# rgiordan/LinearResponseVariationalBayes.py

Hardware: AMD Instinct MI355X
Metric: ELBO-Hessian builds/sec, N=1e+06 obs x D=1024 free params (higher is better)
Workload: dtype f64

## Files before the change

### linearresponsevariationalbayes.py_amd/csrc/k_wsyrk.hip

```cpp
#include "lrvb_internal.h"
#include <type_traits>
#include <math.h>

typedef double d4 __attribute__((ext_vector_type(4)));
typedef double d2 __attribute__((ext_vector_type(2)));

constexpr int WS_LDS_STRIDE = WS_TILE + 16;

int wsyrk_num_tiles(i64 P) {
    i64 nb = (P + WS_TILE - 1) / WS_TILE;
    return (int)(nb * (nb + 1) / 2);
}

int wsyrk_auto_splits(const lrvb_ctx* c) {
    if (c->n_splits_user > 0) return ((c->n_splits_user + 7) / 8) * 8;
    int T = wsyrk_num_tiles(c->P);
    i64 s = (4608 + T / 2) / T;
    s = ((s + 7) / 8) * 8;
    i64 max_by_rows = c->N / 1900;
    max_by_rows = (max_by_rows / 8) * 8;
    if (s > max_by_rows) s = max_by_rows;
    if (s > 128) s = 128;
    if (s < 8) s = 8;
    return (int)s;
// ... 593 lines not shown

    d4 acc[16];
#pragma unroll
    for (int i = 0; i < 16; ++i) acc[i] = (d4){0.0, 0.0, 0.0, 0.0};
    int ca = bi * WS_TILE + 2 * lane; if (ca > PA - 2) ca = PA - 2;
    int cb = bj * WS_TILE + 2 * lane; if (cb > PB - 2) cb = PB - 2;

    const unsigned lds0 = (unsigned)(uintptr_t)(__attribute__((address_space(3))) double*)lds;
    const unsigned voffA = (unsigned)ca * 8u, voffB = (unsigned)cb * 8u, voffC = (unsigned)lane * 4u;
    const unsigned voffX = (unsigned)(lane < 62 ? lane : 61) * 4u;
    auto issue_stage = [&](int ch, int buf) {
        const unsigned base = lds0 + (unsigned)(buf * WS_BUF) * 8u;
        const i64 n0 = r0 + (i64)ch * WS_KC;
#pragma unroll
        for (int i = 0; i < 4; ++i) {
            const int row = wave + 4 * i;
            i64 n = n0 + row; if (n > N - 1) n = N - 1;
            const unsigned la = base + (unsigned)(row * WS_LDS_STRIDE) * 8u;
            if (SLIVER == 2)
                WS_GLDS4_S(reinterpret_cast<const char*>(A + n * lda), voffX, la + 8u);
            else
                WS_GLDS16_S(reinterpret_cast<const char*>(A + n * lda), voffA, la);
            WS_GLDS16_S(reinterpret_cast<const char*>(B + n * ldb), voffB, la + (unsigned)WS_PANEL * 8u);
        }
        if (wave == 0)
            WS_GLDS4_S(reinterpret_cast<const char*>(cpad + n0), voffC, base + (unsigned)(2 * WS_PANEL) * 8u);
    };
    if (SLIVER == 2) {
        if (tid < 32) lds[(tid >> 4) * WS_BUF + (tid & 15) * WS_LDS_STRIDE] = 1.0;
        __syncthreads();
    }
    if (nch > 0) issue_stage(0, 0);
    __builtin_amdgcn_s_waitcnt(0x0F70);
    __syncthreads();

    const int l15 = lane & 15, l4 = lane >> 4;
    const int wr = wave >> 1, wc = wave & 1;
    int mt_a = (PA - bi * WS_TILE - wr * 64 + 15) / 16; mt_a = mt_a < 0 ? 0 : (mt_a > 4 ? 4 : mt_a);
    int mt_b = (PB - bj * WS_TILE - wc * 64 + 15) / 16; mt_b = mt_b < 0 ? 0 : (mt_b > 4 ? 4 : mt_b);
    mt_a = __builtin_amdgcn_readfirstlane(mt_a); mt_b = __builtin_amdgcn_readfirstlane(mt_b);
    const bool full = (PA - bi * WS_TILE >= WS_TILE) && (PB - bj * WS_TILE >= WS_TILE);
    double* out = partial + ((i64)split * T + t) * (i64)(WS_TILE * WS_TILE);
    if (full) {
        const double* a_base = lds + l4 * WS_LDS_STRIDE + 32 * wave + 2 * l15;
        const double* b_base = lds + WS_PANEL + l4 * WS_LDS_STRIDE + 2 * l15;
        const double* c_base = lds + 2 * WS_PANEL + l4;
        const double* a_base_s = a_base + bj * 4 * WS_LDS_STRIDE;
        const double* b_base_s = b_base + bi * 4 * WS_LDS_STRIDE + 32 * wave;
        const double* c_base_i = c_base + bj * 4;
        const double* c_base_ii = c_base + bi * 4;
        const unsigned voffSA = (unsigned)(((i64)(4 * bi + l4) * lda + 4 * WS_TILE + l15) * 8);
        const unsigned voffSB = (unsigned)(((i64)(4 * bj + l4) * ldb + 4 * WS_TILE + l15) * 8);
        double asl[2] = {0.0, 0.0}, bsl[2] = {0.0, 0.0};
        d4 acc_i0 = (d4){0.0, 0.0, 0.0, 0.0}, acc_i1 = acc_i0, acc_ii0 = acc_i0, acc_ii1 = acc_i0, acc_c = acc_i0;
        auto pair_of = [](int v, int& a, int& b) {
            a = (int)((sqrtf(8.f * (float)v + 1.f) - 1.f) * 0.5f);
            while (a * (a + 1) / 2 > v) --a;
            while ((a + 1) * (a + 2) / 2 <= v) ++a;
            b = v - a * (a + 1) / 2;
        };
        const double *ga0 = lds, *gb0 = lds, *ga1 = lds, *gb1 = lds, *gas = lds, *gbs = lds;
        if (SLIVER == 2) {
            int a, b;
            pair_of(bi * WS_TILE + 32 * wave + 2 * l15, a, b);     ga0 = lds + l4 * WS_LDS_STRIDE + a; gb0 = lds + l4 * WS_LDS_STRIDE + b;
            pair_of(bi * WS_TILE + 32 * wave + 2 * l15 + 1, a, b); ga1 = lds + l4 * WS_LDS_STRIDE + a; gb1 = lds + l4 * WS_LDS_STRIDE + b;
            pair_of(4 * WS_TILE + l15, a, b);
            gas = lds + (4 * bi + l4) * WS_LDS_STRIDE + a; gbs = lds + (4 * bi + l4) * WS_LDS_STRIDE + b;
        }
        const bool corner = SLIVER && (bi == bj) && (wave == 0);
        auto load_sliver = [&](int ch, double& a, double& b) {
            const i64 n0 = r0 + (i64)ch * WS_KC;
            if (SLIVER == 1) asm volatile("global_load_dwordx2 %0, %1, %2" : "+v"(a) : "v"(voffSA), "s"(A + n0 * lda) : "memory");
            asm volatile("global_load_dwordx2 %0, %1, %2" : "+v"(b) : "v"(voffSB), "s"(B + n0 * ldb) : "memory");
        };
        if (SLIVER) {
            load_sliver(0, asl[0], bsl[0]);
            __builtin_amdgcn_s_waitcnt(0x0F70);
            asm volatile("" : "+v"(asl[0]), "+v"(bsl[0]));
        }
        auto stage = [&](auto buf_tag, int ch) {
            constexpr int BUF = decltype(buf_tag)::value;
            double af[2][2], gf[2][2], bf[2][8], cv[2];
            if (SLIVER) load_sliver(ch + 1 < nch ? ch + 1 : ch, asl[BUF ^ 1], bsl[BUF ^ 1]);
            d2 ax = (d2){0.0, 0.0}, bx = (d2){0.0, 0.0};
            double cxi = 0.0, cxii = 0.0;
            double asg = 0.0;
            if (SLIVER) {
                if (SLIVER == 2) {
                    const int os = BUF * WS_BUF + bj * 4 * WS_LDS_STRIDE;
                    ax = (d2){ga0[os] * gb0[os], ga1[os] * gb1[os]};
                    asg = gas[BUF * WS_BUF] * gbs[BUF * WS_BUF];
                } else {
                    ax = *reinterpret_cast<const d2*>(a_base_s + BUF * WS_BUF);
                }
                bx = *reinterpret_cast<const d2*>(b_base_s + BUF * WS_BUF);
                cxi = c_base_i[BUF * WS_BUF]; cxii = c_base_ii[BUF * WS_BUF];
            }
            auto read_frags = [&](int kk, int set) {
                const int o = BUF * WS_BUF + kk * 4 * WS_LDS_STRIDE;
                cv[set] = c_base[BUF * WS_BUF + kk * 4];
                if (SLIVER == 2) {
                    af[set][0] = ga0[o]; af[set][1] = ga1[o]; gf[set][0] = gb0[o]; gf[set][1] = gb1[o];
                } else {
                    const d2 va = *reinterpret_cast<const d2*>(a_base + o);
                    af[set][0] = va[0]; af[set][1] = va[1];
                }
#pragma unroll
                for (int h = 0; h < 4; ++h) {
                    const d2 vb = *reinterpret_cast<const d2*>(b_base + o + 32 * h);
                    bf[set][2 * h] = vb[0]; bf[set][2 * h + 1] = vb[1];
                }
            };
            read_frags(0, 0);
#pragma unroll
            for (int kk = 0; kk < WS_KC / 4; ++kk) {
                const int set = kk & 1;
                const double as0 = (SLIVER == 2 ? af[set][0] * gf[set][0] : af[set][0]) * cv[set];
                const double as1 = (SLIVER == 2 ? af[set][1] * gf[set][1] : af[set][1]) * cv[set];
                __builtin_amdgcn_sched_barrier(0);
                if (kk + 1 < WS_KC / 4) read_frags(kk + 1, set ^ 1);
                __builtin_amdgcn_sched_barrier(0);
#pragma unroll
                for (int n = 0; n < 8; ++n) {
                    acc[n] = __builtin_amdgcn_mfma_f64_16x16x4f64(as0, bf[set][n], acc[n], 0, 0, 0);
                    acc[8 + n] = __builtin_amdgcn_mfma_f64_16x16x4f64(as1, bf[set][n], acc[8 + n], 0, 0, 0);
                }
                if (SLIVER && kk == 1) {
                    const double sa = (SLIVER == 2 ? asg : asl[BUF]) * cxii;
                    acc_i0 = __builtin_amdgcn_mfma_f64_16x16x4f64(ax[0] * cxi, bsl[BUF], acc_i0, 0, 0, 0);
                    acc_i1 = __builtin_amdgcn_mfma_f64_16x16x4f64(ax[1] * cxi, bsl[BUF], acc_i1, 0, 0, 0);
                    acc_ii0 = __builtin_amdgcn_mfma_f64_16x16x4f64(sa, bx[0], acc_ii0, 0, 0, 0);
                    acc_ii1 = __builtin_amdgcn_mfma_f64_16x16x4f64(sa, bx[1], acc_ii1, 0, 0, 0);
                    if (corner) acc_c = __builtin_amdgcn_mfma_f64_16x16x4f64(sa, bsl[BUF], acc_c, 0, 0, 0);
                }
                __builtin_amdgcn_sched_barrier(0);
            }
            __builtin_amdgcn_s_waitcnt(0x0F70);
            if (SLIVER) asm volatile("" : "+v"(asl[BUF ^ 1]), "+v"(bsl[BUF ^ 1]));
            __syncthreads();
        };
        for (int ch = 0; ch < nch; ch += 2) {
            if (ch + 1 < nch) issue_stage(ch + 1, 1);
            stage(std::integral_constant<int, 0>{}, ch);
            if (ch + 1 < nch) {
                if (ch + 2 < nch) issue_stage(ch + 2, 0);
                stage(std::integral_constant<int, 1>{}, ch + 1);
            }
        }
#pragma unroll
        for (int m = 0; m < 2; ++m)
#pragma unroll
            for (int n = 0; n < 8; ++n)
#pragma unroll
                for (int r = 0; r < 4; ++r)
                    out[(32 * wave + 2 * (l4 + 4 * r) + m) * WS_TILE + 32 * (n >> 1) + 2 * l15 + (n & 1)] = acc[m * 8 + n][r];
        if (SLIVER) {
            double* oe = partial + ((i64)split * T + (bi * nbb + 4)) * (i64)(WS_TILE * WS_TILE);
            double* of = partial + ((i64)split * T + (4 * nbb + bj)) * (i64)(WS_TILE * WS_TILE);
#pragma unroll
            for (int r = 0; r < 4; ++r) {
                oe[(32 * wave + 2 * (l4 + 4 * r)) * WS_TILE + 16 * bj + l15] = acc_i0[r];
                oe[(32 * wave + 2 * (l4 + 4 * r) + 1) * WS_TILE + 16 * bj + l15] = acc_i1[r];
                of[(16 * bi + l4 + 4 * r) * WS_TILE + 32 * wave + 2 * l15] = acc_ii0[r];
                of[(16 * bi + l4 + 4 * r) * WS_TILE + 32 * wave + 2 * l15 + 1] = acc_ii1[r];
            }
            if (corner) {
                double* oc = partial + ((i64)split * T + (4 * nbb + 4)) * (i64)(WS_TILE * WS_TILE);
#pragma unroll
                for (int r = 0; r < 4; ++r) oc[(16 * bi + l4 + 4 * r) * WS_TILE + l15] = acc_c[r];
            }
        }
        return;
    }
    int buf = 0;
    for (int ch = 0; ch < nch; ++ch) {
        if (ch + 1 < nch) issue_stage(ch + 1, buf ^ 1);
        const double* As = lds + buf * WS_BUF;
        const double* Bs = As + WS_PANEL;
        const double* Cs = As + 2 * WS_PANEL;
        double af[2][4], bf[2][4], cv[2];
        auto read_frags = [&](int kk, int set) {
            const int krow = kk * 4 + l4;
            cv[set] = Cs[krow];
#pragma unroll
            for (int m = 0; m < 4; ++m) af[set][m] = As[krow * WS_LDS_STRIDE + wr * 64 + m * 16 + l15];
#pragma unroll
            for (int n = 0; n < 4; ++n) bf[set][n] = Bs[krow * WS_LDS_STRIDE + wc * 64 + n * 16 + l15];
        };
        read_frags(0, 0);
#pragma unroll
        for (int kk = 0; kk < WS_KC / 4; ++kk) {
            const int set = kk & 1;
            double as[4];
#pragma unroll
            for (int m = 0; m < 4; ++m) as[m] = af[set][m] * cv[set];
            __builtin_amdgcn_sched_barrier(0);
            if (kk + 1 < WS_KC / 4) read_frags(kk + 1, set ^ 1);
            __builtin_amdgcn_sched_barrier(0);
#pragma unroll
            for (int m = 0; m < 4; ++m)
#pragma unroll
                for (int n = 0; n < 4; ++n)
                    if (m < mt_a && n < mt_b)
                        acc[m * 4 + n] = __builtin_amdgcn_mfma_f64_16x16x4f64(as[m], bf[set][n], acc[m * 4 + n], 0, 0, 0);
            __builtin_amdgcn_sched_barrier(0);
        }
        __builtin_amdgcn_s_waitcnt(0x0F70);
        __syncthreads();
        buf ^= 1;
    }
#pragma unroll
    for (int m = 0; m < 4; ++m)
#pragma unroll
        for (int n = 0; n < 4; ++n)
#pragma unroll
            for (int r = 0; r < 4; ++r)
                out[(wr * 64 + m * 16 + l4 + 4 * r) * WS_TILE + wc * 64 + n * 16 + l15] = acc[m * 4 + n][r];
}

int launch_atb_kron32(lrvb_ctx* c, const double* X31, const double* B, i64 N, const double* cvec_dev, double* C_dev);

__global__ __launch_bounds__(256)
void atb_tiles_to_dense_kernel(const double* __restrict__ tiles, int nbb, i64 PA, i64 PB, double* __restrict__ C, i64 ldc, int sliver)
{
    const i64 j = (i64)blockIdx.x * blockDim.x + threadIdx.x;
    const i64 i = blockIdx.y;
    if (j >= PB || i >= PA) return;
    const i64 ti = i / WS_TILE, tj = j / WS_TILE, li = i % WS_TILE, lj = j % WS_TILE;
    const double* tile = tiles + (ti * nbb + tj) * (WS_TILE * WS_TILE);
    if (!sliver || (ti < 4 && tj < 4)) { C[i * ldc + j] = tile[li * WS_TILE + lj]; return; }
    double s = 0.0;
    if (ti < 4)      for (int g = 0; g < 4; ++g) s += tile[li * WS_TILE + 16 * g + lj];
    else             for (int g = 0; g < 4; ++g) s += tile[(16 * g + li) * WS_TILE + lj];
    C[i * ldc + j] = s;
}

int launch_atb(lrvb_ctx* c, const double* A, i64 PA, const double* B, i64 PB, i64 N,
               const double* cvec_dev, double* C_dev, bool rows_padded) {
    if ((PA % 2) || (PB % 2) || (((uintptr_t)A) & 15) || (((uintptr_t)B) & 15))
        LRVB_FAIL(LRVB_ERR_UNSUPPORTED, "atb: operands must have even widths and 16-byte aligned rows");
    const int nba = (int)((PA + WS_TILE - 1) / WS_TILE), nbb = (int)((PB + WS_TILE - 1) / WS_TILE);
    const int T = nba * nbb;
    const bool sliver = rows_padded && PA == 4 * WS_TILE + 16 && PB == 4 * WS_TILE + 16;
    const int TW = sliver ? 16 : T;
    i64 S = (4608 + TW / 2) / TW;
    S = ((S + 7) / 8) * 8;
    i64 max_by_rows = (N / 256 / 8) * 8;
    if (S > max_by_rows) S = max_by_rows;
    if (S > 128) S = 128;
    if (S < 8) S = 8;
    i64 rps = (N + S - 1) / S;
    rps = ((rps + WS_KC - 1) / WS_KC) * WS_KC;
    const i64 tile_elems = (i64)T * WS_TILE * WS_TILE;
    LRVB_TRY(buf_reserve(c, c->tile_part, (size_t)(tile_elems * (S + 1))));
    double* part = c->tile_part.p;
    double* tiles = c->tile_part.p + tile_elems * S;
    if (c->prof_on) LRVB_TRY(prof_mark(c, PROF_WSYRK));
    if (sliver)
        hipLaunchKernelGGL(atb_glds_kernel<1>, dim3((unsigned)(S * 16)), dim3(WS_THREADS), 0, c->stream,
                           A, PA, (int)PA, B, PB, (int)PB, N, cvec_dev, (int)S, nba, nbb, rps, part);
    else
        hipLaunchKernelGGL(atb_glds_kernel<0>, dim3((unsigned)(S * T)), dim3(WS_THREADS), 0, c->stream,
                           A, PA, (int)PA, B, PB, (int)PB, N, cvec_dev, (int)S, nba, nbb, rps, part);
    HIP_TRY(hipGetLastError());
    if (c->prof_on) LRVB_TRY(prof_mark(c, PROF_WSYRK));
    hipLaunchKernelGGL(wsyrk_reduce_kernel, dim3((unsigned)((tile_elems / 2 + 255) / 256)), dim3(256), 0, c->stream,
                       part, (int)S, tile_elems, tiles);
    HIP_TRY(hipGetLastError());
    dim3 grid((unsigned)((PB + 255) / 256), (unsigned)PA);
    hipLaunchKernelGGL(atb_tiles_to_dense_kernel, grid, dim3(256), 0, c->stream, tiles, nbb, PA, PB, C_dev, PB, sliver ? 1 : 0);
    HIP_TRY(hipGetLastError());
    return LRVB_OK;
}


int launch_atb_kron32(lrvb_ctx* c, const double* X31, const double* B, i64 N, const double* cvec_dev, double* C_dev) {
    const i64 PA = 4 * WS_TILE + 16, PB = PA;
    if ((((uintptr_t)B) & 15) || (((uintptr_t)X31) & 7)) LRVB_FAIL(LRVB_ERR_UNSUPPORTED, "atb: operand alignment");
    const int nba = 5, nbb = 5, T = 25;
    i64 S = 128;
    i64 max_by_rows = (N / 256 / 8) * 8;
    if (S > max_by_rows) S = max_by_rows;
    if (S < 8) S = 8;
    i64 rps = (N + S - 1) / S;
    rps = ((rps + WS_KC - 1) / WS_KC) * WS_KC;
    const i64 tile_elems = (i64)T * WS_TILE * WS_TILE;
    LRVB_TRY(buf_reserve(c, c->tile_part, (size_t)(tile_elems * (S + 1))));
    double* part = c->tile_part.p;
    double* tiles = c->tile_part.p + tile_elems * S;
    if (c->prof_on) LRVB_TRY(prof_mark(c, PROF_WSYRK));
    hipLaunchKernelGGL(atb_glds_kernel<2>, dim3((unsigned)(S * 16)), dim3(WS_THREADS), 0, c->stream,
                       X31, (i64)31, (int)PA, B, PB, (int)PB, N, cvec_dev, (int)S, nba, nbb, rps, part);
    HIP_TRY(hipGetLastError());
    if (c->prof_on) LRVB_TRY(prof_mark(c, PROF_WSYRK));
    hipLaunchKernelGGL(wsyrk_reduce_kernel, dim3((unsigned)((tile_elems / 2 + 255) / 256)), dim3(256), 0, c->stream,
                       part, (int)S, tile_elems, tiles);
    HIP_TRY(hipGetLastError());
    dim3 grid((unsigned)((PB + 255) / 256), (unsigned)PA);
    hipLaunchKernelGGL(atb_tiles_to_dense_kernel, grid, dim3(256), 0, c->stream, tiles, nbb, PA, PB, C_dev, PB, 1);
    HIP_TRY(hipGetLastError());
    return LRVB_OK;
}

constexpr int KR_STRIDE = 176;
constexpr int KR_ZERO = 65;
constexpr int KR_CZ = 80;

__device__ __forceinline__ void kr_pair(int v, int pv, int& a, int& b) {
    if (v >= pv) { a = KR_ZERO; b = KR_ZERO; return; }
    a = (int)((sqrtf(8.f * (float)v + 1.f) - 1.f) * 0.5f);
    while (a * (a + 1) / 2 > v) --a;
    while ((a + 1) * (a + 2) / 2 <= v) ++a;
    b = v - a * (a + 1) / 2;
}

__global__ __launch_bounds__(WS_THREADS, 2)
void wsyrk_kron_kernel(const double* __restrict__ Z, i64 ldz, i64 N, int q, int pv,
                       const double* __restrict__ cpad, int n_splits, int nb, i64 rows_per_split,
                       double* __restrict__ partial)
{
    __shared__ double lds[2 * WS_KC * KR_STRIDE];
    const int tid = threadIdx.x;
    const int lane = tid & 63;
    const int wave = __builtin_amdgcn_readfirstlane(tid >> 6);
    const int xcd = blockIdx.x & 7;
    const int qpos = blockIdx.x >> 3;
    const int S8 = n_splits >> 3;
    const int n_off = nb * (nb - 1) / 2;
    int bi, bj, split_local;
    if (qpos < n_off * S8) {
        split_local = qpos / n_off;
        const int u = qpos - split_local * n_off;
        bi = (int)((1.f + sqrtf(1.f + 8.f * (float)u)) * 0.5f);
        while (bi * (bi - 1) / 2 > u) --bi;
        while ((bi + 1) * bi / 2 <= u) ++bi;
        bj = u - bi * (bi - 1) / 2;
    } else {
        const int qd = qpos - n_off * S8;
        split_local = qd / nb;
        bi = bj = qd - split_local * nb;
    }
    const bool diag = (bi == bj);
    const int t = bi * (bi + 1) / 2 + bj;
    const int T = nb * (nb + 1) / 2;
    const int split = split_local * 8 + xcd;
    i64 r0 = (i64)split * rows_per_split;
    i64 r1 = r0 + rows_per_split;
    if (r1 > N) r1 = N;
    if (r0 > N) r0 = N;
    const int nch = (int)((r1 - r0 + WS_KC - 1) / WS_KC);

    d4 acc[16];
#pragma unroll
    for (int i = 0; i < 16; ++i) acc[i] = (d4){0.0, 0.0, 0.0, 0.0};

    const int srow = tid >> 4, seg = tid & 15;
    double sv[4], sc;
    auto load_stage = [&](int ch) {
        i64 n = r0 + (i64)ch * WS_KC + srow;
        sc = cpad[n];
        if (n > N - 1) n = N - 1;
        const double* rowp = Z + n * ldz;
#pragma unroll
        for (int j = 0; j < 4; ++j) { const int col = 4 * seg + j; sv[j] = rowp[col < q ? col : 0]; }
    };
    auto store_stage = [&](int buf) {
        asm volatile("" : "+v"(sv[0]), "+v"(sv[1]), "+v"(sv[2]), "+v"(sv[3]), "+v"(sc));
        double* dst = lds + buf * (WS_KC * KR_STRIDE) + srow * KR_STRIDE;
#pragma unroll
        for (int j = 0; j < 4; ++j) { const int col = 4 * seg + j; const double zv = col < q ? sv[j] : 0.0; dst[col] = zv; dst[KR_CZ + col] = zv * sc; }
    };
    if (tid < 2 * WS_KC) { lds[tid * KR_STRIDE + KR_ZERO] = 0.0; lds[tid * KR_STRIDE + KR_CZ + KR_ZERO] = 0.0; }

    if (nch > 0) { load_stage(0); store_stage(0); }
    __syncthreads();

    const int l15 = lane & 15, l4 = lane >> 4;
    int buf = 0;
    if (!diag) {
        const int wr = wave >> 1, wc = wave & 1;
        int ia[4], ib[4], ja[4], jb[4];
#pragma unroll
        for (int m = 0; m < 4; ++m) {
            kr_pair(bi * WS_TILE + wr * 64 + 16 * m + l15, pv, ia[m], ib[m]);
            kr_pair(bj * WS_TILE + wc * 64 + 16 * m + l15, pv, ja[m], jb[m]);
        }
        int mt_a = (pv - (bi * WS_TILE + wr * 64) + 15) / 16;
        mt_a = __builtin_amdgcn_readfirstlane(mt_a < 0 ? 0 : (mt_a > 4 ? 4 : mt_a));
        for (int ch = 0; ch < nch; ++ch) {
            const bool more = ch + 1 < nch;
            if (more) load_stage(ch + 1);
            const double* zs = lds + buf * (WS_KC * KR_STRIDE);
            double xa[2][4], xb[2][4], ya[2][4], yb[2][4];
            auto read_frags = [&](int kk, int set) {
                const double* rowp = zs + (kk * 4 + l4) * KR_STRIDE;
#pragma unroll
                for (int m = 0; m < 4; ++m) { xa[set][m] = rowp[KR_CZ + ia[m]]; xb[set][m] = rowp[ib[m]]; ya[set][m] = rowp[ja[m]]; yb[set][m] = rowp[jb[m]]; }
            };
            read_frags(0, 0);
#pragma unroll
            for (int kk = 0; kk < WS_KC / 4; ++kk) {
                const int set = kk & 1;
                double af[4], bf[4];
#pragma unroll
                for (int m = 0; m < 4; ++m) { af[m] = xa[set][m] * xb[set][m]; bf[m] = ya[set][m] * yb[set][m]; }
                __builtin_amdgcn_sched_barrier(0);
                if (kk + 1 < WS_KC / 4) read_frags(kk + 1, set ^ 1);
                __builtin_amdgcn_sched_barrier(0);
                __builtin_amdgcn_s_setprio(1);
#pragma unroll
                for (int m = 0; m < 4; ++m)
#pragma unroll
                    for (int n = 0; n < 4; ++n)
                        if (m < mt_a)
                            acc[m * 4 + n] = __builtin_amdgcn_mfma_f64_16x16x4f64(af[m], bf[n], acc[m * 4 + n], 0, 0, 0);
                __builtin_amdgcn_s_setprio(0);
                __builtin_amdgcn_sched_barrier(0);
            }
            if (more) store_stage(buf ^ 1);
            __syncthreads();
            buf ^= 1;
        }
        double* out = partial + ((i64)split * T + t) * (i64)(WS_TILE * WS_TILE);
#pragma unroll
        for (int m = 0; m < 4; ++m)
#pragma unroll
            for (int n = 0; n < 4; ++n)
#pragma unroll
                for (int r = 0; r < 4; ++r)
                    out[(wr * 64 + m * 16 + l4 + 4 * r) * WS_TILE + wc * 64 + n * 16 + l15] = acc[m * 4 + n][r];
    } else {
        const int rb0 = wave, rb1 = 7 - wave;
        const int nreal = (pv - bi * WS_TILE + 15) / 16;
        int i0a, i0b, i1a, i1b, ja[8], jb[8];
        kr_pair(bi * WS_TILE + 16 * rb0 + l15, pv, i0a, i0b);
        kr_pair(bi * WS_TILE + 16 * rb1 + l15, pv, i1a, i1b);
#pragma unroll
        for (int n = 0; n < 8; ++n) kr_pair(bi * WS_TILE + 16 * n + l15, pv, ja[n], jb[n]);
        for (int ch = 0; ch < nch; ++ch) {
            const bool more = ch + 1 < nch;
            if (more) load_stage(ch + 1);
            const double* zs = lds + buf * (WS_KC * KR_STRIDE);
            double ya[2][8], yb[2][8], a0[2], a1[2];
            auto read_frags = [&](int kk, int set) {
                const double* rowp = zs + (kk * 4 + l4) * KR_STRIDE;
#pragma unroll
                for (int n = 0; n < 8; ++n) { ya[set][n] = rowp[ja[n]]; yb[set][n] = rowp[jb[n]]; }
                a0[set] = rowp[KR_CZ + i0a] * rowp[i0b];
                a1[set] = rowp[KR_CZ + i1a] * rowp[i1b];
            };
            read_frags(0, 0);
#pragma unroll
            for (int kk = 0; kk < WS_KC / 4; ++kk) {
                const int set = kk & 1;
                double bf[8];
#pragma unroll
                for (int n = 0; n < 8; ++n) bf[n] = ya[set][n] * yb[set][n];
                const double af0 = a0[set], af1 = a1[set];
                __builtin_amdgcn_sched_barrier(0);
                if (kk + 1 < WS_KC / 4) read_frags(kk + 1, set ^ 1);
                __builtin_amdgcn_sched_barrier(0);
#pragma unroll
                for (int n = 0; n < 4; ++n)
                    if (n <= rb0 && rb0 < nreal) acc[n] = __builtin_amdgcn_mfma_f64_16x16x4f64(af0, bf[n], acc[n], 0, 0, 0);
#pragma unroll
                for (int n = 0; n < 8; ++n)
                    if (n <= rb1 && rb1 < nreal) acc[4 + n] = __builtin_amdgcn_mfma_f64_16x16x4f64(af1, bf[n], acc[4 + n], 0, 0, 0);
                __builtin_amdgcn_sched_barrier(0);
            }
            if (more) store_stage(buf ^ 1);
            __syncthreads();
            buf ^= 1;
        }
        double* out = partial + ((i64)split * T + t) * (i64)(WS_TILE * WS_TILE);
#pragma unroll
        for (int n = 0; n < 8; ++n)
#pragma unroll
            for (int r = 0; r < 4; ++r) {
                const double v0 = (n < 4 && n <= rb0) ? acc[n < 4 ? n : 0][r] : 0.0;
                const double v1 = (n <= rb1) ? acc[4 + n][r] : 0.0;
                out[(rb0 * 16 + l4 + 4 * r) * WS_TILE + n * 16 + l15] = v0;
                out[(rb1 * 16 + l4 + 4 * r) * WS_TILE + n * 16 + l15] = v1;
            }
    }
}

int launch_wsyrk_kron(lrvb_ctx* c, const double* cvec_dev, double* tiles_out_dev) {
    const int q = (int)c->P;
    if (q > 64) LRVB_FAIL(LRVB_ERR_UNSUPPORTED, "Kronecker Gram kernel supports n_cols <= 64 (got %d)", q);
    const int pv = q * (q + 1) / 2;
    const int nb = (pv + WS_TILE - 1) / WS_TILE;
    const int T = nb * (nb + 1) / 2;
    i64 S = (9216 + T / 2) / T;
    S = ((S + 7) / 8) * 8;
    i64 max_by_rows = (c->N / 256 / 8) * 8;
    if (S > max_by_rows) S = max_by_rows;
    if (S > 128) S = 128;
    if (S < 8) S = 8;
    i64 rps = (c->N + S - 1) / S;
    rps = ((rps + WS_KC - 1) / WS_KC) * WS_KC;
    const i64 tile_elems = (i64)T * WS_TILE * WS_TILE;
    LRVB_TRY(buf_reserve(c, c->tile_part, (size_t)(tile_elems * S)));
    if (c->prof_on) LRVB_TRY(prof_mark(c, PROF_WSYRK));
    hipLaunchKernelGGL(wsyrk_kron_kernel, dim3((unsigned)(S * T)), dim3(WS_THREADS), 0, c->stream,
                       c->X.p, c->P, c->N, q, pv, cvec_dev, (int)S, nb, rps, c->tile_part.p);
    HIP_TRY(hipGetLastError());
    if (c->prof_on) LRVB_TRY(prof_mark(c, PROF_WSYRK));
    const i64 nthreads = tile_elems / 2;
    hipLaunchKernelGGL(wsyrk_reduce_kernel, dim3((unsigned)((nthreads + 255) / 256)), dim3(256), 0, c->stream,
                       c->tile_part.p, (int)S, tile_elems, tiles_out_dev);
    HIP_TRY(hipGetLastError());
    if (c->prof_on) {
        const double pvd = (double)pv;
        c->prof.wsyrk_flops = (double)c->N * pvd * (pvd + 1.0);
        c->prof.wsyrk_bytes = 8.0 * (double)c->N * (q + 1.0) + 8.0 * 0.5 * pvd * (pvd + 1.0);
    }
    return LRVB_OK;
}

__global__ __launch_bounds__(256)
void wsyrk_reduce_kernel(const double* __restrict__ partial, int n_splits, i64 tile_elems_total,
                         double* __restrict__ tiles)
{
    const i64 e2 = ((i64)blockIdx.x * blockDim.x + threadIdx.x) * 2;
    if (e2 >= tile_elems_total) return;
    double s0 = 0.0, s1 = 0.0;
    typedef double v2d __attribute__((ext_vector_type(2)));
    for (int s = 0; s < n_splits; ++s) {
        const v2d v = __builtin_nontemporal_load(reinterpret_cast<const v2d*>(partial + (i64)s * tile_elems_total + e2));
        s0 += v[0]; s1 += v[1];
    }
    *reinterpret_cast<double2*>(tiles + e2) = make_double2(s0, s1);
}

__global__ __launch_bounds__(512)
void rpart_reduce_kernel(const double* __restrict__ rpart, int n_splits, i64 width, i64 P, double* __restrict__ r)
{
    __shared__ double sh[8][64];
    const int cx = threadIdx.x & 63, ry = threadIdx.x >> 6;
    const i64 p = (i64)blockIdx.x * 64 + cx;
    double s0 = 0.0, s1 = 0.0;
    if (p < P) {
        int k = ry;
        for (; k + 8 < n_splits; k += 16) { s0 += rpart[(i64)k * width + p]; s1 += rpart[(i64)(k + 8) * width + p]; }
        for (; k < n_splits; k += 8) s0 += rpart[(i64)k * width + p];
    }
    sh[ry][cx] = s0 + s1;
    __syncthreads();
    if (ry == 0 && p < P) {
        double t = sh[0][cx];
#pragma unroll
        for (int g = 1; g < 8; ++g) t += sh[g][cx];
        r[p] = t;
    }
}

bool wsyrk_fast_path(const lrvb_ctx* c) {
    return c->P > 64 && (c->P % 2) == 0 && ((((uintptr_t)c->X.p) & 15) == 0) && !c->force_generic_wsyrk;
}

int launch_wsyrk(lrvb_ctx* c, const double* cvec_dev, double* tiles_out_dev) {
    return launch_wsyrk_r(c, cvec_dev, tiles_out_dev, nullptr, nullptr);
}

int launch_wsyrk_r(lrvb_ctx* c, const double* cvec_dev, double* tiles_out_dev, const double* cy_dev, double* r_out_dev) {
    if (cy_dev && !wsyrk_fast_path(c)) LRVB_FAIL(LRVB_ERR_UNSUPPORTED, "the column sums ride on the LDS-DMA SYRK kernel only");
    if (c->P <= 64 && !c->force_generic_wsyrk)
        return launch_gram_small(c, cvec_dev, tiles_out_dev);
    const int T = wsyrk_num_tiles(c->P);
    const int S = wsyrk_auto_splits(c);
    i64 rps = (c->N + S - 1) / S;
    rps = ((rps + WS_KC - 1) / WS_KC) * WS_KC;
    if (rps < WS_KC) rps = WS_KC;
    const i64 tile_elems = (i64)T * WS_TILE * WS_TILE;
    const int nbt = (int)((c->P + WS_TILE - 1) / WS_TILE);
    const i64 rwidth = (i64)nbt * WS_TILE;
    LRVB_TRY(buf_reserve(c, c->tile_part, (size_t)(tile_elems * S) + (size_t)(rwidth * S)));
    double* rpart = c->tile_part.p + tile_elems * S;
    const i64 ldx = c->P;
    const int vec_ok = ((ldx % 2) == 0) && ((((uintptr_t)c->X.p) & 15) == 0);
    const int grid = S * T;
    if (c->prof_on) LRVB_TRY(prof_mark(c, PROF_WSYRK));
    if (vec_ok && c->P >= 2 && !c->force_generic_wsyrk)
        hipLaunchKernelGGL(wsyrk_glds_kernel, dim3(grid), dim3(WS_THREADS), 0, c->stream,
                           c->X.p, ldx, c->N, (int)c->P, cvec_dev, S, nbt, rps, c->tile_part.p, cy_dev, rpart);
    else if (vec_ok)
        hipLaunchKernelGGL(wsyrk_kernel<true>, dim3(grid), dim3(WS_THREADS), 0, c->stream,
                           c->X.p, ldx, c->N, (int)c->P, cvec_dev, S, T, rps, c->tile_part.p);
    else
        hipLaunchKernelGGL(wsyrk_kernel<false>, dim3(grid), dim3(WS_THREADS), 0, c->stream,
                           c->X.p, ldx, c->N, (int)c->P, cvec_dev, S, T, rps, c->tile_part.p);
    HIP_TRY(hipGetLastError());
    if (c->prof_on) LRVB_TRY(prof_mark(c, PROF_WSYRK));
    const i64 nthreads = tile_elems / 2;
    hipLaunchKernelGGL(wsyrk_reduce_kernel, dim3((unsigned)((nthreads + 255) / 256)), dim3(256), 0, c->stream,
                       c->tile_part.p, S, tile_elems, tiles_out_dev);
    HIP_TRY(hipGetLastError());
    if (cy_dev && r_out_dev) {
        hipLaunchKernelGGL(rpart_reduce_kernel, dim3((unsigned)((c->P + 63) / 64)), dim3(512), 0, c->stream,
                           rpart, S, rwidth, c->P, r_out_dev);
        HIP_TRY(hipGetLastError());
    }
    if (c->prof_on) {
        c->prof.wsyrk_flops = (double)c->N * (double)c->P * (double)(c->P + 1);
        c->prof.wsyrk_bytes = 8.0 * ((double)c->N * (double)(c->P + 1)) + 8.0 * 0.5 * (double)c->P * (double)(c->P + 1);
    }
    return LRVB_OK;
}

__global__ __launch_bounds__(256)
void tiles_to_dense_kernel(const double* __restrict__ tiles, i64 P, double* __restrict__ dense,
                           i64 ld, i64 row_off, i64 col_off, int accumulate)
{
    const i64 j = (i64)blockIdx.x * blockDim.x + threadIdx.x;
    const i64 i = blockIdx.y;
    if (j >= P || i >= P) return;
    const i64 a = i > j ? i : j, b = i > j ? j : i;
    const i64 ba = a / WS_TILE, bb = b / WS_TILE;
    const i64 t = ba * (ba + 1) / 2 + bb;
    const double v = tiles[t * (WS_TILE * WS_TILE) + (a % WS_TILE) * WS_TILE + (b % WS_TILE)];
    double* dst = dense + (row_off + i) * ld + col_off + j;
    if (accumulate) *dst += v; else *dst = v;
}

int launch_tiles_to_dense(lrvb_ctx* c, const double* tiles_dev, i64 P, double* dense_dev, i64 ld,
                          i64 row_off, i64 col_off, bool accumulate) {
    if (P <= 0) return LRVB_OK;
    dim3 grid((unsigned)((P + 255) / 256), (unsigned)P);
    hipLaunchKernelGGL(tiles_to_dense_kernel, grid, dim3(256), 0, c->stream,
                       tiles_dev, P, dense_dev, ld, row_off, col_off, accumulate ? 1 : 0);
    HIP_TRY(hipGetLastError());
    return LRVB_OK;
}

__global__ __launch_bounds__(256)
void wsyrk_batched_reduce_kernel(const double* __restrict__ partial, int n_splits, i64 tile_elems, double* __restrict__ tiles)
{
    const i64 e = (i64)blockIdx.x * blockDim.x + threadIdx.x;
    if (e >= tile_elems) return;
    const i64 g = blockIdx.y;
    const double* src = partial + g * (i64)n_splits * tile_elems + e;
    double s = 0.0;
    for (int k = 0; k < n_splits; ++k) s += __builtin_nontemporal_load(src + (i64)k * tile_elems);
    tiles[g * tile_elems + e] = s;
}

bool wsyrk_batched_supported(const lrvb_ctx* c) { return wsyrk_fast_path(c); }

int launch_wsyrk_batched(lrvb_ctx* c, const double* cols, i64 cstride, int G, double* tiles_out) {
    if (!wsyrk_batched_supported(c)) LRVB_FAIL(LRVB_ERR_UNSUPPORTED, "batched SYRK: even P > 64, 16-byte aligned X");
    if (G <= 0) return LRVB_OK;
    const int T = wsyrk_num_tiles(c->P);
    const i64 Teff = (i64)T * G;
    i64 S = (4608 + Teff / 2) / Teff;
    S = ((S + 7) / 8) * 8;
    i64 max_by_rows = (c->N / 1900 / 8) * 8;
    if (S > max_by_rows) S = max_by_rows;
    if (S > 128) S = 128;
    if (S < 8) S = 8;
    i64 rps = (c->N + S - 1) / S;
    rps = ((rps + WS_KC - 1) / WS_KC) * WS_KC;
    if (rps < WS_KC) rps = WS_KC;
    const i64 tile_elems = (i64)T * WS_TILE * WS_TILE;
    LRVB_TRY(buf_reserve(c, c->tile_part, (size_t)(tile_elems * S * G)));
    const int nbt = (int)((c->P + WS_TILE - 1) / WS_TILE);
    if (c->prof_on) LRVB_TRY(prof_mark(c, PROF_WSYRK));
    hipLaunchKernelGGL(wsyrk_glds_batched_kernel, dim3((unsigned)(S * T), (unsigned)G), dim3(WS_THREADS), 0, c->stream,
                       c->X.p, c->P, c->N, (int)c->P, cols, cstride, (int)S, nbt, rps, c->tile_part.p, tile_elems * S);
    HIP_TRY(hipGetLastError());
    if (c->prof_on) LRVB_TRY(prof_mark(c, PROF_WSYRK));
    hipLaunchKernelGGL(wsyrk_batched_reduce_kernel, dim3((unsigned)((tile_elems + 255) / 256), (unsigned)G), dim3(256), 0, c->stream,
                       (const double*)c->tile_part.p, (int)S, tile_elems, tiles_out);
    HIP_TRY(hipGetLastError());
    return LRVB_OK;
}
```

Baseline: 65.11.

## Pre-form Kronecker product panels in LDS with a three-stage pipeline

The Kronecker Gram kernel now has each wave gather raw Z row entries and compute the pairwise products once per row into packed LDS panels, rather than every MFMA lane recomputing products from scattered LDS reads. A pipeline runs global load, raw-row staging, and panel formation for the next chunk while MFMAs consume the current panel. Fragment reads become vectorised d2 loads, and full chunks use precomputed byte offsets instead of per-row clamping. The cost is more LDS, more pipeline bookkeeping, and a reworked wave-to-output mapping that must remain correct for partial tiles.

```diff
diff --git a/linearresponsevariationalbayes.py_amd/csrc/k_wsyrk.hip b/linearresponsevariationalbayes.py_amd/csrc/k_wsyrk.hip
--- a/linearresponsevariationalbayes.py_amd/csrc/k_wsyrk.hip
+++ b/linearresponsevariationalbayes.py_amd/csrc/k_wsyrk.hip
@@ -919,12 +919,16 @@
     return LRVB_OK;
 }
 
-constexpr int KR_STRIDE = 176;
-constexpr int KR_ZERO = 65;
-constexpr int KR_CZ = 80;
+constexpr int KP_PANEL = WS_KC * WS_TILE;
+constexpr int KP_BUF = 2 * KP_PANEL;
+constexpr int KZ_STRIDE = 82;
+constexpr int KZ_ZERO = 64;
+constexpr int KZ_C = 66;
+constexpr int KZ_BASE = 2 * KP_BUF;
+constexpr int KR_LDS = KZ_BASE + WS_KC * KZ_STRIDE;
 
 __device__ __forceinline__ void kr_pair(int v, int pv, int& a, int& b) {
-    if (v >= pv) { a = KR_ZERO; b = KR_ZERO; return; }
+    if (v >= pv) { a = KZ_ZERO; b = KZ_ZERO; return; }
     a = (int)((sqrtf(8.f * (float)v + 1.f) - 1.f) * 0.5f);
     while (a * (a + 1) / 2 > v) --a;
     while ((a + 1) * (a + 2) / 2 <= v) ++a;
@@ -936,7 +940,7 @@
                        const double* __restrict__ cpad, int n_splits, int nb, i64 rows_per_split,
                        double* __restrict__ partial)
 {
-    __shared__ double lds[2 * WS_KC * KR_STRIDE];
+    __shared__ __attribute__((aligned(16))) double lds[KR_LDS];
     const int tid = threadIdx.x;
     const int lane = tid & 63;
     const int wave = __builtin_amdgcn_readfirstlane(tid >> 6);
@@ -971,125 +975,186 @@
 #pragma unroll
     for (int i = 0; i < 16; ++i) acc[i] = (d4){0.0, 0.0, 0.0, 0.0};
 
-    const int srow = tid >> 4, seg = tid & 15;
+    const int srow = 4 * wave + (lane >> 4), seg = lane & 15;
+    unsigned zoff[4];
+#pragma unroll
+    for (int j = 0; j < 4; ++j) { const int col = 4 * seg + j; zoff[j] = (unsigned)(((i64)srow * ldz + (col < q ? col : 0)) * 8); }
+    const unsigned coff = (unsigned)srow * 8u;
+    i64 full = (N - r0) / WS_KC;
+    const int nch_full = (int)(full < nch ? full : nch);
     double sv[4], sc;
     auto load_stage = [&](int ch) {
-        i64 n = r0 + (i64)ch * WS_KC + srow;
-        sc = cpad[n];
-        if (n > N - 1) n = N - 1;
-        const double* rowp = Z + n * ldz;
-#pragma unroll
-        for (int j = 0; j < 4; ++j) { const int col = 4 * seg + j; sv[j] = rowp[col < q ? col : 0]; }
+        const i64 n0 = r0 + (i64)ch * WS_KC;
+        if (ch < nch_full) {
+            const char* zb = reinterpret_cast<const char*>(Z) + n0 * ldz * 8;
+            const char* cb = reinterpret_cast<const char*>(cpad + n0);
+#pragma unroll
+            for (int j = 0; j < 4; ++j) sv[j] = *reinterpret_cast<const double*>(zb + zoff[j]);
+            sc = *reinterpret_cast<const double*>(cb + coff);
+        } else {
+            i64 n = n0 + srow;
+            sc = cpad[n < N ? n : N];
+            if (n > N - 1) n = N - 1;
+            const char* zb = reinterpret_cast<const char*>(Z) + (n - srow) * ldz * 8;
+#pragma unroll
+            for (int j = 0; j < 4; ++j) sv[j] = *reinterpret_cast<const double*>(zb + zoff[j]);
+        }
     };
-    auto store_stage = [&](int buf) {
+    double* zrow_w = lds + KZ_BASE + srow * KZ_STRIDE;
+    auto store_stage = [&]() {
         asm volatile("" : "+v"(sv[0]), "+v"(sv[1]), "+v"(sv[2]), "+v"(sv[3]), "+v"(sc));
-        double* dst = lds + buf * (WS_KC * KR_STRIDE) + srow * KR_STRIDE;
-#pragma unroll
-        for (int j = 0; j < 4; ++j) { const int col = 4 * seg + j; const double zv = col < q ? sv[j] : 0.0; dst[col] = zv; dst[KR_CZ + col] = zv * sc; }
+        *reinterpret_cast<d2*>(zrow_w + 4 * seg) = (d2){sv[0], sv[1]};
+        *reinterpret_cast<d2*>(zrow_w + 4 * seg + 2) = (d2){sv[2], sv[3]};
+        zrow_w[KZ_C + seg] = sc;
     };
-    if (tid < 2 * WS_KC) { lds[tid * KR_STRIDE + KR_ZERO] = 0.0; lds[tid * KR_STRIDE + KR_CZ + KR_ZERO] = 0.0; }
-
-    if (nch > 0) { load_stage(0); store_stage(0); }
+    if (lane < 4) lds[KZ_BASE + (4 * wave + lane) * KZ_STRIDE + KZ_ZERO] = 0.0;
+
+    const double* zw = lds + KZ_BASE + 4 * wave * KZ_STRIDE;
+    const double *ga[4], *gb[4];
+    {
+        int a, b;
+#pragma unroll
+        for (int e = 0; e < 4; ++e) {
+            kr_pair((e < 2 ? bi : bj) * WS_TILE + 64 * (e & 1) + lane, pv, a, b);
+            ga[e] = zw + a; gb[e] = zw + b;
+        }
+    }
+    const double* gc = zw + KZ_C;
+    double* pw = lds + 4 * wave * WS_TILE + 2 * lane;
+    double g[8], gck;
+    auto gather = [&](int row) {
+        if (!diag) {
+#pragma unroll
+            for (int e = 0; e < 4; ++e) { g[2 * e] = ga[e][row * KZ_STRIDE]; g[2 * e + 1] = gb[e][row * KZ_STRIDE]; }
+        } else {
+#pragma unroll
+            for (int e = 0; e < 2; ++e) { g[2 * e] = ga[e][row * KZ_STRIDE]; g[2 * e + 1] = gb[e][row * KZ_STRIDE]; }
+        }
+        gck = gc[row * KZ_STRIDE];
+    };
+    auto form = [&](int row, int nbuf) {
+        double* dst = pw + nbuf * KP_BUF + row * WS_TILE;
+        if (!diag) {
+            *reinterpret_cast<d2*>(dst) = (d2){(g[0] * g[1]) * gck, (g[2] * g[3]) * gck};
+            *reinterpret_cast<d2*>(dst + KP_PANEL) = (d2){g[4] * g[5], g[6] * g[7]};
+        } else {
+            *reinterpret_cast<d2*>(dst) = (d2){g[0] * g[1], g[2] * g[3]};
+            dst[KP_PANEL - lane] = gck;
+        }
+    };
+
+    load_stage(0); store_stage();
     __syncthreads();
+#pragma unroll
+    for (int row = 0; row < 4; ++row) { gather(row); form(row, 0); }
+    load_stage(1); store_stage();
+    __syncthreads();
 
     const int l15 = lane & 15, l4 = lane >> 4;
-    int buf = 0;
+    double* out = partial + ((i64)split * T + t) * (i64)(WS_TILE * WS_TILE);
     if (!diag) {
-        const int wr = wave >> 1, wc = wave & 1;
-        int ia[4], ib[4], ja[4], jb[4];
-#pragma unroll
-        for (int m = 0; m < 4; ++m) {
-            kr_pair(bi * WS_TILE + wr * 64 + 16 * m + l15, pv, ia[m], ib[m]);
-            kr_pair(bj * WS_TILE + wc * 64 + 16 * m + l15, pv, ja[m], jb[m]);
-        }
-        int mt_a = (pv - (bi * WS_TILE + wr * 64) + 15) / 16;
-        mt_a = __builtin_amdgcn_readfirstlane(mt_a < 0 ? 0 : (mt_a > 4 ? 4 : mt_a));
-        for (int ch = 0; ch < nch; ++ch) {
-            const bool more = ch + 1 < nch;
-            if (more) load_stage(ch + 1);
-            const double* zs = lds + buf * (WS_KC * KR_STRIDE);
-            double xa[2][4], xb[2][4], ya[2][4], yb[2][4];
+        const int nreal = (pv - bi * WS_TILE + 15) / 16;
+        const bool m0 = __builtin_amdgcn_readfirstlane(wave < nreal), m1 = __builtin_amdgcn_readfirstlane(wave + 4 < nreal);
+        const double* a_base = lds + l4 * WS_TILE + 32 * wave + 2 * l15;
+        const double* b_base = lds + KP_PANEL + l4 * WS_TILE + 2 * l15;
+        auto stage = [&](auto buf_tag) {
+            constexpr int BUF = decltype(buf_tag)::value;
+            d2 af[2], bf[2][4];
             auto read_frags = [&](int kk, int set) {
-                const double* rowp = zs + (kk * 4 + l4) * KR_STRIDE;
-#pragma unroll
-                for (int m = 0; m < 4; ++m) { xa[set][m] = rowp[KR_CZ + ia[m]]; xb[set][m] = rowp[ib[m]]; ya[set][m] = rowp[ja[m]]; yb[set][m] = rowp[jb[m]]; }
+                const int o = BUF * KP_BUF + kk * 4 * WS_TILE;
+                af[set] = *reinterpret_cast<const d2*>(a_base + o);
+#pragma unroll
+                for (int h = 0; h < 4; ++h) bf[set][h] = *reinterpret_cast<const d2*>(b_base + o + 32 * h);
             };
             read_frags(0, 0);
 #pragma unroll
             for (int kk = 0; kk < WS_KC / 4; ++kk) {
                 const int set = kk & 1;
-                double af[4], bf[4];
-#pragma unroll
-                for (int m = 0; m < 4; ++m) { af[m] = xa[set][m] * xb[set][m]; bf[m] = ya[set][m] * yb[set][m]; }
                 __builtin_amdgcn_sched_barrier(0);
                 if (kk + 1 < WS_KC / 4) read_frags(kk + 1, set ^ 1);
+                gather(kk);
                 __builtin_amdgcn_sched_barrier(0);
                 __builtin_amdgcn_s_setprio(1);
-#pragma unroll
-                for (int m = 0; m < 4; ++m)
-#pragma unroll
-                    for (int n = 0; n < 4; ++n)
-                        if (m < mt_a)
-                            acc[m * 4 + n] = __builtin_amdgcn_mfma_f64_16x16x4f64(af[m], bf[n], acc[m * 4 + n], 0, 0, 0);
+                if (m0) {
+#pragma unroll
+                    for (int n = 0; n < 8; ++n) acc[n] = __builtin_amdgcn_mfma_f64_16x16x4f64(af[set][0], bf[set][n >> 1][n & 1], acc[n], 0, 0, 0);
+                }
+                if (m1) {
+#pragma unroll
+                    for (int n = 0; n < 8; ++n) acc[8 + n] = __builtin_amdgcn_mfma_f64_16x16x4f64(af[set][1], bf[set][n >> 1][n & 1], acc[8 + n], 0, 0, 0);
+                }
                 __builtin_amdgcn_s_setprio(0);
                 __builtin_amdgcn_sched_barrier(0);
-            }
-            if (more) store_stage(buf ^ 1);
+                form(kk, BUF ^ 1);
+                __builtin_amdgcn_sched_barrier(0);
+            }
+            store_stage();
             __syncthreads();
-            buf ^= 1;
-        }
-        double* out = partial + ((i64)split * T + t) * (i64)(WS_TILE * WS_TILE);
-#pragma unroll
-        for (int m = 0; m < 4; ++m)
-#pragma unroll
-            for (int n = 0; n < 4; ++n)
+        };
+        for (int ch = 0; ch < nch; ch += 2) {
+            load_stage(ch + 2);
+            stage(std::integral_constant<int, 0>{});
+            if (ch + 1 < nch) {
+                load_stage(ch + 3);
+                stage(std::integral_constant<int, 1>{});
+            }
+        }
+#pragma unroll
+        for (int m = 0; m < 2; ++m)
+#pragma unroll
+            for (int n = 0; n < 8; ++n)
 #pragma unroll
                 for (int r = 0; r < 4; ++r)
-                    out[(wr * 64 + m * 16 + l4 + 4 * r) * WS_TILE + wc * 64 + n * 16 + l15] = acc[m * 4 + n][r];
+                    out[(16 * wave + 64 * m + l4 + 4 * r) * WS_TILE + 16 * (n >> 1) + 64 * (n & 1) + l15] = acc[m * 8 + n][r];
     } else {
         const int rb0 = wave, rb1 = 7 - wave;
         const int nreal = (pv - bi * WS_TILE + 15) / 16;
-        int i0a, i0b, i1a, i1b, ja[8], jb[8];
-        kr_pair(bi * WS_TILE + 16 * rb0 + l15, pv, i0a, i0b);
-        kr_pair(bi * WS_TILE + 16 * rb1 + l15, pv, i1a, i1b);
-#pragma unroll
-        for (int n = 0; n < 8; ++n) kr_pair(bi * WS_TILE + 16 * n + l15, pv, ja[n], jb[n]);
-        for (int ch = 0; ch < nch; ++ch) {
-            const bool more = ch + 1 < nch;
-            if (more) load_stage(ch + 1);
-            const double* zs = lds + buf * (WS_KC * KR_STRIDE);
-            double ya[2][8], yb[2][8], a0[2], a1[2];
+        const double* p_base = lds + l4 * WS_TILE + 2 * l15;
+        const double* a0_base = p_base + 32 * rb0;
+        const double* a1_base = p_base + 32 * (rb1 - 4) + 1;
+        const double* c_base = lds + KP_PANEL + l4 * WS_TILE;
+        auto stage = [&](auto buf_tag) {
+            constexpr int BUF = decltype(buf_tag)::value;
+            double a0[2], a1[2], cv[2];
+            d2 bf[2][4];
             auto read_frags = [&](int kk, int set) {
-                const double* rowp = zs + (kk * 4 + l4) * KR_STRIDE;
-#pragma unroll
-                for (int n = 0; n < 8; ++n) { ya[set][n] = rowp[ja[n]]; yb[set][n] = rowp[jb[n]]; }
-                a0[set] = rowp[KR_CZ + i0a] * rowp[i0b];
-                a1[set] = rowp[KR_CZ + i1a] * rowp[i1b];
+                const int o = BUF * KP_BUF + kk * 4 * WS_TILE;
+                cv[set] = c_base[o];
+                a0[set] = a0_base[o];
+                a1[set] = a1_base[o];
+#pragma unroll
+                for (int h = 0; h < 4; ++h) bf[set][h] = *reinterpret_cast<const d2*>(p_base + o + 32 * h);
             };
             read_frags(0, 0);
 #pragma unroll
             for (int kk = 0; kk < WS_KC / 4; ++kk) {
                 const int set = kk & 1;
-                double bf[8];
-#pragma unroll
-                for (int n = 0; n < 8; ++n) bf[n] = ya[set][n] * yb[set][n];
-                const double af0 = a0[set], af1 = a1[set];
+                const double s0 = a0[set] * cv[set], s1 = a1[set] * cv[set];
                 __builtin_amdgcn_sched_barrier(0);
                 if (kk + 1 < WS_KC / 4) read_frags(kk + 1, set ^ 1);
+                gather(kk);
                 __builtin_amdgcn_sched_barrier(0);
 #pragma unroll
                 for (int n = 0; n < 4; ++n)
-                    if (n <= rb0 && rb0 < nreal) acc[n] = __builtin_amdgcn_mfma_f64_16x16x4f64(af0, bf[n], acc[n], 0, 0, 0);
+                    if (n <= rb0 && rb0 < nreal) acc[n] = __builtin_amdgcn_mfma_f64_16x16x4f64(s0, bf[set][n][0], acc[n], 0, 0, 0);
 #pragma unroll
                 for (int n = 0; n < 8; ++n)
-                    if (n <= rb1 && rb1 < nreal) acc[4 + n] = __builtin_amdgcn_mfma_f64_16x16x4f64(af1, bf[n], acc[4 + n], 0, 0, 0);
-                __builtin_amdgcn_sched_barrier(0);
-            }
-            if (more) store_stage(buf ^ 1);
+                    if (n <= rb1 && rb1 < nreal) acc[4 + n] = __builtin_amdgcn_mfma_f64_16x16x4f64(s1, bf[set][n & 3][n >> 2], acc[4 + n], 0, 0, 0);
+                __builtin_amdgcn_sched_barrier(0);
+                form(kk, BUF ^ 1);
+                __builtin_amdgcn_sched_barrier(0);
+            }
+            store_stage();
             __syncthreads();
-            buf ^= 1;
-        }
-        double* out = partial + ((i64)split * T + t) * (i64)(WS_TILE * WS_TILE);
+        };
+        for (int ch = 0; ch < nch; ch += 2) {
+            load_stage(ch + 2);
+            stage(std::integral_constant<int, 0>{});
+            if (ch + 1 < nch) {
+                load_stage(ch + 3);
+                stage(std::integral_constant<int, 1>{});
+            }
+        }
 #pragma unroll
         for (int n = 0; n < 8; ++n)
 #pragma unroll
```

After: 65.02. About the same (-0.1%).
